# SahakyanLab/GenomeAssembler_dev

Hardware: AMD Instinct MI355X
Metric: k-mers built+scored/sec (higher is better)
Workload: dtype u64 keys / u32 counts / f64 scores; 1 GPU; cfg2 (configs[2]): 100 x 50000 bp segments per GPU, 150 bp reads at 50x, k=31, build + breakage scoring of all contigs; mode=segments, segments_total=100, distinct_kmers_rank0=3843627, parallelism=segments sharded over 1 GPU(s), no collective

## Files before the change

### genomeassembler_dev_amd/csrc/capi.hip

```cpp
#include <algorithm>
#include <atomic>
#include <functional>
#include <memory>
#include <mutex>
#include <new>
#include <thread>

#include "pipeline.h"
#include "scaffolds.h"

struct gasm_strlist {
    std::vector<char> data;
    std::vector<u64> off;
};

struct gasm_contigs {
    std::vector<char> data;
    std::vector<u64> off;
    u64 rows = 0;
    std::vector<u32> perm;
    int words = 1;
    std::vector<u64> dkeys;
    std::vector<u32> dmult;
};
// ... 40 lines not shown
        StepSlot& x = slot[cur];
        if (!x.cx) x.cx = cur ? ctx->lane((size_t)cur) : ctx;
        if (!x.cx) x.cx = ctx;
        return x;
    }
    const StepSlot& S() const { return slot[cur]; }
    bool built = false;
    bool scored = false;
    int score_kmer = 0;
    u32 score_tables = 1;
    int last_k = 0;
    DBuf d_read_start;
    std::vector<u32> h_read_start;
    std::vector<int64_t> h_fx;
    std::vector<u64> h_sim_seg_off;
    DBuf d_rkc;
    bool rkc_checked = false;
    bool rkc_counted = false;
    std::vector<u32> h_rkc;
};

static int batch_queue_score(gasm_batch* b, StepSlot& x) {
    ScoreTable* tbs[GASM_MAX_TABLES];
    b->table_ptrs(tbs);
    return pipeline_score_launch(x.cx, b->rd, x.dp, b->score_kmer, tbs, b->score_tables, false, false, x.ss, &x.bs);
}

static int batch_finish(gasm_batch* b) {
    StepSlot& x = b->S();
    bool rebuilt = false;
    GCHK(pipeline_build_finish(x.cx, b->build_reads(x), x.bs, &rebuilt));
    if (rebuilt) {
        x.paths_ready = false;
        if (b->scored) {
            GCHK(pipeline_contig_paths(x.cx, b->rd, x.bs, x.dp));
            x.paths_ready = true;
            pipeline_contig_paths_host(b->rd, x.bs, x.dp);
            GCHK(batch_queue_score(b, x));
        }
    }
    return GASM_OK;
}

static void strlist_from(const std::vector<std::string>& v, std::vector<char>& data, std::vector<u64>& off) {
    off.assign(v.size() + 1, 0);
    size_t tot = 0;
    for (size_t i = 0; i < v.size(); ++i) { tot += v[i].size(); off[i + 1] = tot; }
    data.resize(tot);
    for (size_t i = 0; i < v.size(); ++i) memcpy(data.data() + off[i], v[i].data(), v[i].size());
}

template <class F>
static int new_batch(gasm_ctx* ctx, u32 n_segments, u64 n_reads, gasm_batch** out, F&& fill) {
    gasm_batch* b = new gasm_batch();
    b->ctx = ctx;
    b->n_segments = n_segments;
    b->n_reads = n_reads;
    const int st = fill(b);
    if (st != GASM_OK) { gasm_batch_free(b); return st; }
    *out = b;
    return GASM_OK;
}

extern "C" {

static int breakscore_impl(gasm_ctx* ctx, DevPaths& dp, const std::function<std::string(u64)>& path_text, uint64_t n_paths, const char* reads,
// ... 972 lines not shown
```

### genomeassembler_dev_amd/csrc/kernels.h

```cpp
#pragma once
#include <hip/hip_runtime.h>
#include <stdint.h>

#include "device_utils.h"
#include "keyops.h"

struct ReadSet {
    const u64* words;
    const u64* read_off;
    const u64* seg_read_off;
    const u32* seg_tile_start;
    const uint4* tile_info;
    u32 fixed_len;
    u32 n_segments;
};

__device__ __forceinline__ void read_span(const ReadSet& rs, u64 r, u64* p0, u32* len) {
    if (rs.fixed_len) { *p0 = rs.read_off ? rs.read_off[r] : r * rs.fixed_len; *len = rs.fixed_len; }
    else { const u64 a = rs.read_off[r]; *p0 = a; *len = (u32)(rs.read_off[r + 1] - a); }
}

struct GraphView {
    const void* dk_key;
    const u32* dstart;
// ... 144 lines not shown
    const u32* elem_skip;
    const u64* elem_pos;
};
__global__ void k_str_bitonic(const u64* words, const u64* off, u32* idx, u32 n_pow2, u32 kk, u32 j, ChainSigs cs);
__global__ void k_str_bitonic_block(const u64* words, const u64* off, u32* idx, u32 n_pow2, u32 kk, u32 j0, ChainSigs cs);
__global__ void k_str_adjacent_eq(const u64* words, const u64* off, const u32* idx, u32 n, u8* same_as_prev, ChainSigs cs);
__global__ void k_unpack_ascii(const u64* words, u64 nbases, u8* out);
__global__ void k_guided_chain(PathSet ps, const unsigned long long* fx, int k, u32* g_next, u32* g_prev, u32* dbg_order);
__global__ void k_asm_match(const u64* cwords, const u64* c_off, u32 n, int k, u8* match, u8* row_any, u8* level_any);
__global__ void k_asm_merge(const u32* perm, u32 rows, u32 n, int k, const u32* clen, const u8* match, const u8* row_any, const u8* level_any,
                            const u64* cwords, const u64* c_off, u32* out_next, u8* out_ov, u32* out_heads, u32* out_nchains, u8* need_host);

__global__ void k_sim_weights(const u64* gwords, const u64* gbase, const u64* woff, u32 n_segments, int kmer, const long long* fixw, u64* w);
template <class T> __global__ void k_seg_scan_incl(T* a, const u64* off);
__global__ void k_sim_draw(const u64* cum, const u64* woff, const u64* doff, const u64* glen, u64 seed, u32 read_len, u32* start, u32* keep);
__global__ void k_sim_compact(const u32* start, const u32* keep, const u32* rank, const u64* doff, const u64* seg_read_off, u32* kept_start);
__global__ void k_sim_extract(const u64* gwords, const u64* gbase, const u64* seg_read_off, const u32* kept_start, u32 read_len, unsigned long long* out);

template <int LS>
__global__ void k_read_kmer_count(const u64* words, const u64* read_off, const u64* seg_read_off, u32 fixed_len, u32 n_segments, u32* out);

struct SeedTable {
    u64* seed;
    u32* gpos;
    const u64* tbl_off;
};
__global__ void k_read_insert(ReadSet rs, SeedTable st, int w);
__global__ void k_path_scan(ReadSet rs, PathSet ps, SeedTable st, const u64* seg_base_off, int w, const u64* first_off, u32* first, u32 seg0,
                            u32 path_lo, u32 path_hi);
__global__ void k_first_to_poscnt(const u32* first, u64 n, u32* poscnt);
#define GASM_SCORE_MAX_TABLES 8
struct FixTables { const long long* p[GASM_SCORE_MAX_TABLES]; };
struct ProbTables { const double* p[GASM_SCORE_MAX_TABLES]; };
template <class K, int T>
__global__ void k_score_reads_graph(ReadSet rs, GraphView gv, const u64* link, const u32* e_cid, PathSet ps, FixTables dfix, int kmer,
                                    u32 reads_per_wg, u32 chunks, u32 lds_paths, u32* cnt, unsigned long long* sum, u64 sum_stride, int verify,
                                    u32* verify_flag);
__global__ void k_levenshtein(PathSet ps, u32 n_paths, const u64* twords, u32 nt, int infix, u8* carry_ws, u64 carry_stride, int32_t* out);
__global__ void k_levenshtein2(PathSet ps, u32 n_paths, const u64* twords, u32 nt, int infix, uint4* carry_ws, u64 carry_stride, int32_t* out);
__global__ void k_score_zero(u32* cnt, unsigned long long* sum, u64 sum_stride, u32 n_tables, const u32* n_paths_p);
__global__ void k_score_finish(PathSet ps, const u32* cnt, const unsigned long long* sum, const long long* dfix, const u64* seg_empty,
                               int kmer, double inv_scale, double* bp_score, double* norm_freq, double* norm_len, int32_t* kmer_breaks,
                               int32_t* seq_len, const u32* n_paths_p);
template <int T>
__global__ void k_path_reduce(PathSet ps, const u32* poscnt, const u32* extra, ProbTables dprob, int kmer, double* bp_score, double* norm_freq,
                              double* norm_len, u64 out_stride, int32_t* kmer_breaks, int32_t* seq_len, u32 n_paths);
__global__ void k_path_freq(PathSet ps, const u32* poscnt, const u32* total, const int32_t* drow, int kmer, u32 n_table,
                            u32* freq_cnt, u32 n_paths);
__global__ void k_ks_genome_hist(const u64* gwords, u64 glen, int kmer, const int32_t* drow, u32* hist);
__global__ void k_path_ks(PathSet ps, const u32* poscnt, const int32_t* drow, int kmer, u32 n_table, const double* pv, const u32* cumy, u32* scratch,
                          double* out, u32 n_paths, const u32* list);
__global__ void k_path_ks2(PathSet ps, const u32* poscnt, const int32_t* drow, int kmer, u32 n_table, const double* pv, const u32* cumy, const u32* run_end,
                           u32* scratch, double* out, u32* flags, u32 n_paths, u32 bins);
__global__ void k_cover_mark(const long long* start, const long long* len, u64 n, long long seq_len, int* diff);
__global__ void k_cover_count(const int* diff, long long seq_len, unsigned long long* covered);
__global__ void k_prob_dist(PathSet ps, const double* dprob, int kmer, const u64* pd_off, double* out, u32 n_paths);

template <class T>
struct XReport {
    T* w;
    u32 W;
    __host__ __device__ T& send_tot(u32 d) const { return w[d]; }
    __host__ __device__ T& recv_tot(u32 d) const { return w[W + d]; }
    __host__ __device__ T& info(u32 j) const { return w[2 * W + j]; }
    __host__ __device__ T& flags() const { return w[2 * W + 4]; }
    __host__ __device__ T& ticket() const { return w[2 * W + 5]; }
    static size_t words(u32 W) { return 2 * (size_t)W + 6; }
};
__global__ void k_x_flag_word(const u32* flags, u32* row_tail);
__global__ void k_x1_plan(const u32* lens_all, u64 stride, u32 nbt, const u32* order, const u32* dst_first, const u32* mine, u32 n_mine, u32 W, u32 r, u32 limit,
                          u64* send_off, u64* send_tot, u64* run_off, u32* run_len, u64* recv_tot, u64* bstart, u32* flags_or);
__global__ void k_x2_fill(u32* G, u32 nbt, const u32* mine, u32 n_mine, const u32* bucket_d, const u32* flags);
__global__ void k_x2_plan(const u32* G, const u16* own1, u32 W, u32 r, u32 gb_lo, u32 n_out, int bbits, const u32* mine, u32 n_mine, const u32* seg_first,
                          u64* send_off, u64* send_tot, u64* run_off, u32* run_len, u64* recv_tot, u64* bstart, u64* info);
__global__ void k_x_report(const u64* send_tot, const u64* recv_tot, u32 W, const u64* info, u32 n_info, const u32* flags_or, u64* report, u64 ticket);
__global__ void k_x_add_u32(u32* acc, const u32* v, u64 n);
// ... 1 lines not shown
```

### genomeassembler_dev_amd/csrc/kernels_score.hip

```cpp
#include "device_utils.h"
#include "kernels.h"

#define GASM_DIRECT_ROWS 87380
__device__ __forceinline__ u32 direct_base(u32 L) { return ((1u << (2 * L)) - 4u) / 3u; }

__device__ __forceinline__ bool break_window(const u64* __restrict__ words, u64 pbase, u32 plen, u32 j, int kmer, u32* idx) {
    const int st = (int)j - kmer / 2;
    const u32 start = st > 0 ? (u32)st : 0u;
    u32 width = 8;
    if (start == 0) {
        if (j == 1) width = 2;
        else if (j == 2) width = 4;
        else if (j == 3) width = 6;
    }
    if (start >= plen) return false;
    const u32 avail = plen - start;
    const u32 wd = width < avail ? width : avail;
    *idx = direct_base(wd) + (u32)kmer_at(words, pbase + start, (int)wd);
    return true;
}

__global__ void __launch_bounds__(GASM_WG) k_read_insert(ReadSet rs, SeedTable st, int w) {
    const u32 seg = blockIdx.y;
    const u64 r = rs.seg_read_off[seg] + (u64)blockIdx.x * GASM_WG + threadIdx.x;
// ... 84 lines not shown
}

template <class K>
__device__ __forceinline__ u64 graph_match(const ReadSet& rs, const GraphView& gv, const u64* __restrict__ link,
                                           const u32* __restrict__ e_cid, const PathSet& ps, u32 seg, u64 r, u32* path, u64* pbeg, u64* pend,
                                           int verify, u32* __restrict__ verify_flag) {
    u64 p0; u32 len;
    read_span(rs, r, &p0, &len);
    if (len < (u32)gv.k) return ~0ull;
    const K key = kmer_key_at<K>(rs.words, p0, gv.k);
    u32 hi;
    const u32 e = graph_lower_bound<K>(gv, seg, key, &hi);
    if (e >= hi || !keq(reinterpret_cast<const K*>(gv.dk_key)[e], key)) return ~0ull;
    const u64 l = link[e];
    const u32 a = (u32)(l >> 32);
    if (a == GASM_NONE32 || !(l & GASM_LINK_DONE)) return ~0ull;
    const u32 c = e_cid[a];
    *path = c;
    const gasm_u64x2 po = load_pair(ps.p_off + c);
    *pbeg = po.x; *pend = po.y;
    const u64 g = po.x + ((u32)l & 0x7FFFFFFFu);
    if (g + len > po.y) return ~0ull;
    if (verify) {
        if (!bases_equal(rs.words, p0, ps.words, g, len)) { if (verify == 1) atomicOr(verify_flag, 1u); return ~0ull; }
    }
    return g;
}

template <class K, int T>
__global__ void __launch_bounds__(GASM_WG) k_score_reads_graph(ReadSet rs, GraphView gv, const u64* __restrict__ link,
                                                               const u32* __restrict__ e_cid, PathSet ps, FixTables dfix, int kmer,
                                                               u32 reads_per_wg, u32 chunks, u32 lds_paths, u32* __restrict__ cnt,
                                                               unsigned long long* __restrict__ sum, u64 sum_stride, int verify,
                                                               u32* __restrict__ verify_flag) {
    extern __shared__ unsigned long long s_sum[];
    u32* s_cnt = reinterpret_cast<u32*>(s_sum + (size_t)T * lds_paths);
    u32 seg, chunk;
    if (!seg_chunk(rs.n_segments, chunks, &seg, &chunk)) return;
    const u64 r0 = rs.seg_read_off[seg] + (u64)chunk * reads_per_wg;
    const u64 rseg_end = rs.seg_read_off[seg + 1];
    if (r0 >= rseg_end) return;
    const u64 r1 = r0 + reads_per_wg < rseg_end ? r0 + reads_per_wg : rseg_end;
    const u32 pfirst = ps.seg_path_off[seg], np = ps.seg_path_off[seg + 1] - pfirst;
    const bool in_lds = np <= lds_paths;
    if (in_lds) for (u32 i = threadIdx.x; i < np; i += GASM_WG) {
#pragma unroll
        for (int t = 0; t < T; ++t) s_sum[(size_t)t * lds_paths + i] = 0;
        s_cnt[i] = 0;
    }
    __syncthreads();
    for (u64 r = r0 + threadIdx.x; r < r1; r += GASM_WG) {
        u32 c = 0;
        u64 pb = 0, pe = 0;
        const u64 g = graph_match<K>(rs, gv, link, e_cid, ps, seg, r, &c, &pb, &pe, verify, verify_flag);
        if (g == ~0ull) continue;
        const u32 plen = (u32)(pe - pb);
        u32 idx = 0;
        const bool hit = break_window(ps.words, pb, plen, (u32)(g - pb), kmer, &idx);
        long long fx[T];
#pragma unroll
        for (int t = 0; t < T; ++t) fx[t] = hit ? dfix.p[t][idx] : 0;
        if (in_lds) {
            atomicAdd(&s_cnt[c - pfirst], 1u);
#pragma unroll
            for (int t = 0; t < T; ++t) atomicAdd(&s_sum[(size_t)t * lds_paths + (c - pfirst)], (unsigned long long)fx[t]);
        } else {
            atomicAdd(&cnt[c], 1u);
#pragma unroll
            for (int t = 0; t < T; ++t) atomicAdd(&sum[(u64)t * sum_stride + c], (unsigned long long)fx[t]);
        }
    }
    __syncthreads();
    if (in_lds) for (u32 i = threadIdx.x; i < np; i += GASM_WG) {
        const u32 c = s_cnt[i];
        if (c) {
            atomicAdd(&cnt[pfirst + i], c);
#pragma unroll
            for (int t = 0; t < T; ++t) atomicAdd(&sum[(u64)t * sum_stride + pfirst + i], s_sum[(size_t)t * lds_paths + i]);
        }
    }
}

#define GASM_INST_SCORE(K, T)                                                                                                         \
    template __global__ void k_score_reads_graph<K, T>(ReadSet, GraphView, const u64*, const u32*, PathSet, FixTables, int, u32, u32, u32, u32*, \
                                                       unsigned long long*, u64, int, u32*);
#define GASM_INST_SCORE_K(K)                                                                                                           \
    GASM_INST_SCORE(K, 1) GASM_INST_SCORE(K, 2) GASM_INST_SCORE(K, 3) GASM_INST_SCORE(K, 4) GASM_INST_SCORE(K, 5) GASM_INST_SCORE(K, 6) \
    GASM_INST_SCORE(K, 7) GASM_INST_SCORE(K, 8)
GASM_INST_SCORE_K(u64)
GASM_INST_SCORE_K(K128)

__global__ void __launch_bounds__(GASM_WG) k_score_zero(u32* __restrict__ cnt, unsigned long long* __restrict__ sum, u64 sum_stride, u32 n_tables,
                                                        const u32* __restrict__ n_paths_p) {
    const u32 n = *n_paths_p;
    for (u32 p = blockIdx.x * GASM_WG + threadIdx.x; p < n; p += gridDim.x * GASM_WG) {
        cnt[p] = 0;
        for (u32 t = 0; t < n_tables; ++t) sum[(u64)t * sum_stride + p] = 0;
    }
}

__global__ void __launch_bounds__(GASM_WG) k_score_finish(PathSet ps, const u32* __restrict__ cnt, const unsigned long long* __restrict__ sum,
                                                          const long long* __restrict__ dfix, const u64* __restrict__ seg_empty,
                                                          int kmer, double inv_scale, double* __restrict__ bp_score,
                                                          double* __restrict__ norm_freq, double* __restrict__ norm_len,
                                                          int32_t* __restrict__ kmer_breaks, int32_t* __restrict__ seq_len,
                                                          const u32* __restrict__ n_paths_p) {
    const u32 n_paths = *n_paths_p;
    for (u32 p = blockIdx.x * GASM_WG + threadIdx.x; p < n_paths; p += gridDim.x * GASM_WG) {
        const u64 pb = ps.p_off[p];
        const u32 len = (u32)(ps.p_off[p + 1] - pb);
        u32 tot = cnt[p];
        long long fs = (long long)sum[p];
        if (seg_empty) {
            const u32 seg = upper_seg<u32>(ps.seg_path_off, ps.n_segments, p);
            const u32 e = (u32)seg_empty[seg];
            if (e) {
                u32 idx;
                tot += e;
                if (break_window(ps.words, pb, len, 0, kmer, &idx)) fs += (long long)e * dfix[idx];
            }
        }
        const double s1 = (double)fs * inv_scale;
        bp_score[p] = s1;
        norm_freq[p] = tot ? s1 / (double)tot : 0.0;
        norm_len[p] = s1 / (double)(int32_t)len;
        kmer_breaks[p] = (int32_t)tot;
        seq_len[p] = (int32_t)len;
    }
}

__device__ __forceinline__ u32 wave_sum_u32(u32 v) {
#pragma unroll
    for (int d = 32; d > 0; d >>= 1) v += __shfl_xor(v, d, 64);
    return v;
}

__device__ __forceinline__ double wave_sum_fixed(double v) {
#pragma unroll
    for (int d = 32; d > 0; d >>= 1) v += __shfl_xor(v, d, 64);
    return v;
}

template <int T>
__global__ void __launch_bounds__(GASM_WG) k_path_reduce(PathSet ps, const u32* __restrict__ poscnt, const u32* __restrict__ extra, ProbTables dprob,
                                                         int kmer, double* __restrict__ bp_score, double* __restrict__ norm_freq,
                                                         double* __restrict__ norm_len, u64 out_stride, int32_t* __restrict__ kmer_breaks,
                                                         int32_t* __restrict__ seq_len, u32 n_paths) {
    __shared__ u32 s_t[4];
    __shared__ double s_a[T][4], s_b[T][4];
    const u32 p = blockIdx.x;
    if (p >= n_paths) return;
    const u32 lane = threadIdx.x & 63, wv = threadIdx.x >> 6;
    const u64 pb = ps.p_off[p];
    const u32 len = (u32)(ps.p_off[p + 1] - pb);
    u32 tsum = 0;
    for (u32 j = threadIdx.x; j < len; j += GASM_WG) tsum += poscnt[pb + j];
    tsum = wave_sum_u32(tsum);
    if (lane == 0) s_t[wv] = tsum;
    __syncthreads();
    const u32 tot = s_t[0] + s_t[1] + s_t[2] + s_t[3] + extra[p];
    const double dtot = (double)tot;
    double s1[T], s2[T];
// ... 622 lines not shown
```

### genomeassembler_dev_amd/csrc/pipeline.h

```cpp
#pragma once
#include "gasm_internal.h"
#include "kernels.h"

template <class K> struct KeyTag { using type = K; };
template <class F> static inline int with_key(int words, F&& f) { return words == 1 ? f(KeyTag<u64>{}) : f(KeyTag<K128>{}); }
#define GLAUNCH_K(ctx, words, name, kern, grid, block, shmem, ...)          \
    GCHK(with_key(words, [&](auto _tag) -> int {                            \
        using K = typename decltype(_tag)::type;                            \
        GLAUNCH(ctx, name, kern, grid, block, shmem, __VA_ARGS__);          \
        return GASM_OK;                                                     \
    }))

struct DevReads {
    u32 n_segments = 0;
    u64 n_reads = 0, total_bases = 0;
    u32 fixed_len = 0;
    u32 min_len = 0, max_len = 0;
    u64 n_empty = 0;
    std::vector<u64> h_read_off;
    std::vector<u64> h_seg_read_off;
    std::vector<u64> h_seg_empty;
    bool positioned = false;
    int sim_shift = 52;
    u64 upload_id = 0;
// ... 87 lines not shown
    std::vector<u32> h_dk_cnt, h_nxt;
    std::vector<u64> h_solid_before, h_solid_after, h_spectrum;
    bool spectrum_queued = false;
    std::vector<u8> h_eflag;
    std::vector<char> h_contigs;
    bool fetched_distinct = false, fetched_contigs = false;
    void release();
};

struct ScoreTable {
    DBuf d_prob, d_row, d_fix;
    std::vector<double> h_prob;
    std::vector<double> h_row_prob;
    double h_absmax = 0;
    bool h_finite = false;
    int fix_shift = -1;
    u32 n_table = 0;
    int fixed_shift(u64 max_terms) const;
    int set_fixed(gasm_ctx* ctx, int shift);
    int set(gasm_ctx* ctx, const char* bp_kmer, const u64* bp_off, u64 n_table, const double* bp_prob);
    int set_standard(gasm_ctx* ctx, const double* table69904);
    void release();
};

struct ScoreState {
    DBuf d_tbl_off, d_seed, d_gpos, d_poscnt, d_total, d_out_f64, d_out_i32, d_freq, d_pd_off, d_pd, d_seg_empty, d_fxsum, d_first, d_first_off;
    std::vector<u64> h_toff;
    u32 n_paths = 0, n_table = 0;
    u32 n_tables = 1;
    size_t stride = 1;
    const BuildState* graph = nullptr;
    bool want_freq = false, want_pd = false, launched = false;
    bool verify = false;
    std::vector<double> h_bp, h_nf, h_nl, h_freq, h_pd;
    std::vector<int32_t> h_breaks, h_len;
    std::vector<u64> h_pd_off;
    bool valid = false;
    void release();
};

int pipeline_build(gasm_ctx* ctx, DevReads& rd, int k, u64 genome_len_hint, BuildState& bs, u32 min_count = 1, u32 strands = 1, u32 tip_len = 0,
                   u32 tip_rounds = 0);
int pipeline_build_finish(gasm_ctx* ctx, DevReads& rd, BuildState& bs, bool* rebuilt);
int pipeline_build_finish_n(gasm_ctx* ctx, DevReads* rd, u32 n_segments, BuildState& bs, bool* rebuilt);
enum : u32 { GASM_RUNG_EXACT = 1, GASM_RUNG_TABLE = 2, GASM_RUNG_BBITS = 4, GASM_RUNG_MULTI = 8, GASM_RUNG_ALL = 15 };
bool build_next_config(u32 ovf, u32 rungs, int words, int bb_cap, bool& single_pass, bool& small_tbl, int& bbits, bool& multi_pass);
void pipeline_build_plan(const DevReads& rd, const BuildState& bs, int32_t* row);
int plan_build(gasm_ctx* ctx, DevReads& rd, int k, u64 hint, BuildState& bs);
void distinct_caps(BuildState& bs, u32 n_segments);
int launch_distinct(gasm_ctx* ctx, DevReads& rd, BuildState& bs);
int launch_graph(gasm_ctx* ctx, u32 n_segments, BuildState& bs);
int pipeline_fetch_distinct(gasm_ctx* ctx, DevReads& rd, BuildState& bs);
int pipeline_fetch_contigs(gasm_ctx* ctx, DevReads& rd, BuildState& bs);
int pipeline_fetch_solid_stats(gasm_ctx* ctx, DevReads& rd, BuildState& bs);
int pipeline_fetch_tip_stats(gasm_ctx* ctx, DevReads& rd, BuildState& bs);
int pipeline_kmer_spectrum(gasm_ctx* ctx, DevReads& rd, BuildState& bs);
int pipeline_fetch_kmer_spectrum(gasm_ctx* ctx, DevReads& rd, BuildState& bs);
int pipeline_fetch_contig_twins(gasm_ctx* ctx, DevReads& rd, BuildState& bs);
int pipeline_fetch_graph(gasm_ctx* ctx, DevReads& rd, BuildState& bs);
int pipeline_contig_paths(gasm_ctx* ctx, const DevReads& rd, const BuildState& bs, DevPaths& dp);
void pipeline_contig_paths_host(const DevReads& rd, const BuildState& bs, DevPaths& dp);
int pipeline_score_launch(gasm_ctx* ctx, DevReads& rd, DevPaths& dp, int kmer, ScoreTable* const* tbs, u32 n_tables, bool want_freq,
                          bool want_pd, ScoreState& ss, const BuildState* graph);
int pipeline_score_fetch(gasm_ctx* ctx, ScoreState& ss);
bool pipeline_score_uses_graph(const DevReads& rd, const BuildState& graph, ScoreTable* const* tbs, u32 n_tables);
int pipeline_ks(gasm_ctx* ctx, DevPaths& dp, ScoreState& ss, const ScoreTable& tb, const char* genome, u64 genome_len, int kmer, std::vector<double>& ks);
// ... 16 lines not shown
```

### genomeassembler_dev_amd/csrc/pipeline.hip

```cpp
#include <atomic>
#include <chrono>
#include <thread>
#include "pipeline.h"

#include <algorithm>
#include <cmath>

__global__ void k_set_u64(u64* p, u64 v) { *p = v; }

__global__ void k_add_empty_reads(PathSet ps, const u64* __restrict__ seg_empty, u32* __restrict__ poscnt, u32* __restrict__ total) {
    const u32 seg = blockIdx.y;
    const u32 p = ps.seg_path_off[seg] + blockIdx.x * GASM_WG + threadIdx.x;
    if (p >= ps.seg_path_off[seg + 1]) return;
    const u32 e = (u32)seg_empty[seg];
    if (!e) return;
    if (ps.p_off[p + 1] > ps.p_off[p]) poscnt[ps.p_off[p]] += e;
    else total[p] += e;
}

struct Knobs {
    int dedup_tbl = 0, dbg_dedup = 0, padm = -1, scatter_wgs = 8, hist_wgs = 64, rank_rounds = 18, bbits_add = 0, ruler_shift = 0;
    bool rank_global = false, sync_build = false;
    int dedup_warm = 0;
    const char* stamps = nullptr;
// ... 366 lines not shown
    }
    total_bases = h_p_off[np];
    if (total_bases >= 0xFFFFFFF0ull) { gasm_set_error("paths exceed 2^32 bases"); return GASM_ERR_CAPACITY; }
    h_seg_path_off = {0u, np};
    DBuf ascii;
    GCHK(h2d(ctx, ascii, data + off[0], total_bases));
    int st = pack_from_device_ascii(ctx, ascii.as<u8>());
    ascii.release();
    GCHK(st);
    return upload_dirs(ctx);
}

PathSet DevPaths::view() const {
    PathSet v;
    v.words = d_words.as<u64>();
    v.p_off = b_p_off ? b_p_off : d_p_off.as<u64>();
    v.seg_path_off = b_seg_path_off ? b_seg_path_off : d_seg_path_off.as<u32>();
    v.n_segments = n_segments;
    return v;
}

void DevPaths::release() { d_words.release(); d_p_off.release(); d_seg_path_off.release(); d_seg_base_off.release(); }

void BuildState::release() {
    for (DBuf* b : {&d_solid_removed, &d_tip_stats, &d_spectrum, &d_twin, &d_keys, &d_keys2, &d_mult, &d_hist, &d_toff, &d_tcnt, &d_fdir, &d_bstart, &d_bucket_d, &d_dstart, &d_flags, &d_dk_key, &d_dk_cnt,
                    &d_eflag, &d_nxt, &d_link, &d_clen, &d_ecid, &d_ecoff, &d_rtab, &d_seg_cbases, &d_seg_cstart,
                    &d_seg_bstart, &d_c_off, &d_contig_ascii})
        b->release();
    part_valid = false;
    if (h_report) { (void)hipHostFree(h_report); h_report = nullptr; h_report_words = 0; }
}

void ScoreState::release() {
    for (DBuf* b : {&d_tbl_off, &d_seed, &d_gpos, &d_poscnt, &d_total, &d_out_f64, &d_out_i32, &d_freq, &d_pd_off, &d_pd, &d_seg_empty, &d_fxsum, &d_first, &d_first_off}) b->release();
}

static int ensure_lds_attrs(gasm_ctx* ctx) {
    if (ctx->lds_attrs_set) return GASM_OK;
#define GASM_LDS_ATTR(kern, bytes) HIPCHK(hipFuncSetAttribute(reinterpret_cast<const void*>(kern), hipFuncAttributeMaxDynamicSharedMemorySize, bytes));
#define GASM_SCORE_LDS_ATTR(T) GASM_LDS_ATTR((k_score_reads_graph<K, T>), GASM_SCORE_PATH_CAP * 12)
    for (int words = 1; words <= 2; ++words)
        GCHK(with_key(words, [&](auto tag) -> int {
            using K = typename decltype(tag)::type;
            GASM_LDS_ATTR(k_bucket_scatter<K>, 160 * 1024) GASM_LDS_ATTR(k_bucket_partition<K>, 160 * 1024) GASM_LDS_ATTR(k_tile_hist<K>, 160 * 1024)
            GASM_SCORE_LDS_ATTR(1) GASM_SCORE_LDS_ATTR(2) GASM_SCORE_LDS_ATTR(3) GASM_SCORE_LDS_ATTR(4) GASM_SCORE_LDS_ATTR(5) GASM_SCORE_LDS_ATTR(6) GASM_SCORE_LDS_ATTR(7) GASM_SCORE_LDS_ATTR(8)
            return GASM_OK;
        }));
    GASM_LDS_ATTR(k_rank_lds, 160 * 1024 - 64)
#undef GASM_SCORE_LDS_ATTR
#undef GASM_LDS_ATTR
    ctx->lds_attrs_set = true;
    return GASM_OK;
}

void distinct_caps(BuildState& bs, u32 S) {
    const u64 limit = bs.multi_pass ? GASM_BUCKET_MAX : bs.small_tbl ? GASM_TBL_LIMIT / 2 : GASM_TBL_LIMIT;
    const u64 per_seg = ((u64)1 << bs.bbits) * limit;
    const u64 all = bs.k < 16 ? ((u64)1 << (2 * bs.k)) : ~(u64)0;
    bs.D_cap = 0; bs.maxD_cap = 0;
    for (u32 s = 0; s < S; ++s) {
        const u64 c = std::min(std::min(bs.h_seg_nk[s], per_seg), all);
        bs.D_cap += c;
        bs.maxD_cap = std::max(bs.maxD_cap, c);
    }
}

static int launch_graph_dense(gasm_ctx* ctx, u32 S, BuildState& bs, bool last_pass);
// ... 794 lines not shown
    HIPCHK(hipMemcpyAsync(&c, cov.p, 8, hipMemcpyDeviceToHost, ctx->stream));
    HIPCHK(hipStreamSynchronize(ctx->stream));
    *percent = (1.0 - (double)(seq_len - (long long)c) / (double)seq_len) * 100.0;
    return GASM_OK;
}

static u64 max_seg_reads(const DevReads& rd) {
    u64 m = 0;
    for (u32 s = 0; s < rd.n_segments; ++s) m = std::max(m, rd.h_seg_read_off[s + 1] - rd.h_seg_read_off[s]);
    return m;
}

static_assert(GASM_SCORE_MAX_TABLES == GASM_MAX_TABLES, "kernels.h and gasm.h disagree on the number of tables");

#define GASM_TABLES_SWITCH(T, CASE)                                                                                      \
    switch (T) {                                                                                                         \
        case 1: CASE(1); break; case 2: CASE(2); break; case 3: CASE(3); break; case 4: CASE(4); break; case 5: CASE(5); break;  \
        case 6: CASE(6); break; case 7: CASE(7); break; default: CASE(8); break;                                         \
    }

static int score_launch_graph(gasm_ctx* ctx, DevReads& rd, DevPaths& dp, int kmer, ScoreTable* const* tbs, u32 T, ScoreState& ss,
                              const BuildState& graph) {
    GasmRange range("gasm:score (graph-indexed)");
    GCHK(ensure_lds_attrs(ctx));
    const u32 S = rd.n_segments;
    const size_t PC = (size_t)graph.D_cap + 1;
    ss.stride = PC;
    ss.graph = &graph;
    ss.n_paths = 0;
    const size_t fx_off = (PC * 4 + 15) & ~(size_t)15;
    GCHK(ss.d_total.ensure(fx_off + PC * 8 * T));
    GCHK(ss.d_out_f64.ensure(PC * 8 * 3 * T));
    GCHK(ss.d_out_i32.ensure(PC * 4 * 2));
    unsigned long long* const d_fx = reinterpret_cast<unsigned long long*>(static_cast<char*>(ss.d_total.p) + fx_off);
    const u32* const n_paths_p = graph.d_seg_cstart.as<u32>() + S;
    const u64 p_est = graph.have_actual ? std::max<u64>(graph.n_contigs, 1) : (u64)S * 256;
    const u32 grid_p = (u32)std::max<u64>(1, std::min<u64>(ceil_div_u64(p_est, GASM_WG), (u64)ctx->n_cu * 8));
    GLAUNCH(ctx, "k_score_zero", k_score_zero, dim3(grid_p), dim3(GASM_WG), 0, ss.d_total.as<u32>(), d_fx, (u64)PC, T, n_paths_p);
    const PathSet ps = dp.view();
    const GraphView gv = graph_view(graph);
    const u64 max_reads = max_seg_reads(rd);
    FixTables ft = {};
    for (u32 t = 0; t < T; ++t) {
        GCHK(tbs[t]->set_fixed(ctx, tbs[t]->fixed_shift(max_reads)));
        ft.p[t] = tbs[t]->d_fix.as<long long>();
    }
    const int verify = (graph.min_count > 1 || graph.tip_len) ? 2 : env_int("GASM_SCORE_VERIFY", 0) != 0 ? 1 : 0;
    ss.verify = verify == 1;
    const u32 reads_per_wg = 256;
    const u32 rchunks = (u32)ceil_div_u64(max_reads, reads_per_wg);
    u32 lds_paths = std::min<u32>(std::max<u32>(graph.have_actual ? graph.paths_est : 1024u, 1u), (u32)(GASM_SCORE_PATH_CAP * 12 / (4 + 8 * T)));
    if (const int cap = env_int("GASM_DBG_SCORE_LDS_PATHS", 0)) lds_paths = std::min<u32>(lds_paths, (u32)std::max(1, cap));
    const size_t lds_bytes = (size_t)lds_paths * (4 + 8 * (size_t)T);
#define GASM_LAUNCH_SCORE(TT)                                                                                                                       \
    GLAUNCH_K(ctx, graph.words, "k_score_reads_graph", (k_score_reads_graph<K, TT>), seg_grid(rchunks, S), dim3(GASM_WG), lds_bytes, rd.view(), gv, \
              graph.d_link.as<u64>(), graph.d_ecid.as<u32>(), ps, ft, kmer, reads_per_wg, rchunks, lds_paths, ss.d_total.as<u32>(), d_fx, (u64)PC,  \
              verify, graph.d_flags.as<u32>() + GASM_FLAG_SCORE_MISMATCH)
    GASM_TABLES_SWITCH(T, GASM_LAUNCH_SCORE)
#undef GASM_LAUNCH_SCORE
    int32_t* o_br = ss.d_out_i32.as<int32_t>();
    int32_t* o_ln = o_br + PC;
    const u64* d_se = nullptr;
    if (rd.n_empty) { GCHK(h2d(ctx, ss.d_seg_empty, rd.h_seg_empty.data(), (size_t)S * 8)); d_se = ss.d_seg_empty.as<u64>(); }
    for (u32 t = 0; t < T; ++t) {
        double* o_bp = ss.d_out_f64.as<double>() + (size_t)t * 3 * PC;
        GLAUNCH(ctx, "k_score_finish", k_score_finish, dim3(grid_p), dim3(GASM_WG), 0, ps, ss.d_total.as<u32>(), d_fx + (size_t)t * PC, ft.p[t], d_se, kmer,
                std::ldexp(1.0, -tbs[t]->fix_shift), o_bp, o_bp + PC, o_bp + 2 * PC, o_br, o_ln, n_paths_p);
    }
    ss.h_pd_off.clear();
    ss.launched = true;
    return GASM_OK;
}

bool pipeline_score_uses_graph(const DevReads& rd, const BuildState& graph, ScoreTable* const* tbs, u32 T) {
    if (!(graph.n_kmers > 0 && rd.n_reads > rd.n_empty && rd.min_len >= (u32)graph.k)) return false;
    const u64 max_reads = max_seg_reads(rd);
    for (u32 t = 0; t < T; ++t) if (tbs[t]->fixed_shift(max_reads) < 0) return false;
    return true;
}

static int score_positions(gasm_ctx* ctx, DevReads& rd, DevPaths& dp, ScoreState& ss, u32 n_tables) {
    ss.n_paths = dp.n_paths;
    const u32 S = rd.n_segments, P = dp.n_paths;
    const u64 TB = dp.total_bases;
    ss.stride = (size_t)P + 1;
    GCHK(ss.d_poscnt.ensure((TB + 1) * 4));
    GCHK(ss.d_total.ensure(((size_t)P + 1) * 4));
    GCHK(ss.d_out_f64.ensure(((size_t)P + 1) * 8 * 3 * n_tables));
    GCHK(ss.d_out_i32.ensure(((size_t)P + 1) * 4 * 2));
    HIPCHK(hipMemsetAsync(ss.d_poscnt.p, 0, (TB + 1) * 4, ctx->stream));
    HIPCHK(hipMemsetAsync(ss.d_total.p, 0, ((size_t)P + 1) * 4, ctx->stream));
    const PathSet ps = dp.view();
    const int w = (int)std::min<u32>(32, rd.min_len);
    if (P && TB && rd.n_reads > rd.n_empty && w >= 1) {
        std::vector<u64>& toff = ss.h_toff;
        toff.assign((size_t)S + 1, 0);
        std::vector<u64> foff((size_t)S + 1, 0);
        u64 max_bases = 0, max_reads = 0;
        for (u32 s = 0; s < S; ++s) {
            const u64 nbases = dp.h_seg_base_off[s + 1] - dp.h_seg_base_off[s];
            const u64 nreads = rd.h_seg_read_off[s + 1] - rd.h_seg_read_off[s];
// ... 177 lines not shown
```

### genomeassembler_dev_amd/csrc/pool.hip

```cpp
#include <algorithm>

#include "pool.h"

static int read_lens(gasm_pool* p, u32 n) {
    p->h_len.assign(n, 0);
    if (n) HIPCHK(hipMemcpyAsync(p->h_len.data(), p->bs.d_bucket_d.p, (size_t)n * 4, hipMemcpyDeviceToHost, p->ctx->stream));
    u32 ovf = 0;
    HIPCHK(hipMemcpyAsync(&ovf, p->bs.d_flags.as<u32>() + GASM_FLAG_OVERFLOW, 4, hipMemcpyDeviceToHost, p->ctx->stream));
    HIPCHK(hipStreamSynchronize(p->ctx->stream));
    return (int)(ovf & (GASM_OVF_TABLE | GASM_OVF_REGION));
}

int pool_empty_runs(gasm_pool* p) {
    gasm_ctx* ctx = p->ctx;
    BuildState& bs = p->bs;
    GCHK(bs.d_bucket_d.ensure(((size_t)p->n_runs + 2) * 4));
    GCHK(bs.d_bstart.ensure(((size_t)p->n_runs + 1) * 8));
    GCHK(bs.d_keys.ensure(64)); GCHK(bs.d_mult.ensure(64));
    HIPCHK(hipMemsetAsync(bs.d_bucket_d.p, 0, ((size_t)p->n_runs + 2) * 4, ctx->stream));
    bs.part_valid = false;
    HIPCHK(hipMemsetAsync(bs.d_bstart.p, 0, ((size_t)p->n_runs + 1) * 8, ctx->stream));
    HIPCHK(hipMemsetAsync(bs.d_flags.p, 0, GASM_FLAG_BYTES, ctx->stream));
    return GASM_OK;
}
// ... 49 lines not shown
    if (S == 0) return GASM_OK;
    GCHK(bs.d_dstart.ensure(((size_t)p->n_runs + 2) * 4));
    GLAUNCH(ctx, "k_scan_excl", k_scan_excl<u32>, dim3(1), dim3(1024), 0, bs.d_bucket_d.as<u32>(), bs.d_dstart.as<u32>(), p->n_runs);
    GCHK(launch_graph(ctx, S, bs));
    return GASM_OK;
}

int pool_score_launch(gasm_pool* p, int kmer, const double* table, bool wait_for_build) {
    if (!p->graphed || !p->reads_set) { gasm_set_error("scoring needs the rank's graph and the reads of its segments first"); return GASM_ERR_STATE; }
    gasm_ctx* ctx = p->ctx;
    if (!p->table_set || memcmp(p->table_copy.data(), table, GASM_TABLE_ROWS * sizeof(double)) != 0) {
        GCHK(p->tb.set_standard(ctx, table));
        p->table_copy.assign(table, table + GASM_TABLE_ROWS);
        p->table_set = true;
    }
    ScoreTable* const tb = &p->tb;
    const bool through_graph = p->n_local && pipeline_score_uses_graph(p->own, p->bs, &tb, 1);
    if (wait_for_build || !through_graph) GCHK(pipeline_build_finish_n(ctx, nullptr, p->n_local, p->bs, nullptr));
    if (!p->paths_ready) {
        GCHK(pipeline_contig_paths(ctx, p->own, p->bs, p->dp));
        p->paths_ready = true;
    }
    if (!p->bs.pending) pipeline_contig_paths_host(p->own, p->bs, p->dp);
    GCHK(pipeline_score_launch(ctx, p->own, p->dp, kmer, &tb, 1, false, false, p->ss, &p->bs));
    p->scored = true; p->score_kmer = kmer;
    return GASM_OK;
}

int pool_finish(gasm_pool* p) {
    bool rebuilt = false;
    GCHK(pipeline_build_finish_n(p->ctx, nullptr, p->n_local, p->bs, &rebuilt));
    if (rebuilt && p->scored) {
        p->paths_ready = false;
        GCHK(pool_score_launch(p, p->score_kmer, p->table_copy.data(), true));
    }
    return GASM_OK;
}

extern "C" {

int gasm_pool_create(gasm_ctx* ctx, const char* reads, uint64_t n_reads, uint32_t fixed_len, const uint64_t* seg_read_off,
                     uint32_t n_segments, gasm_pool** out) {
    API_GUARD_BEGIN
    if (!ctx || !out) { gasm_set_error("gasm_pool_create: null argument"); return GASM_ERR_INVALID; }
    *out = nullptr;
    if (fixed_len == 0) { gasm_set_error("pooled builds take fixed-length reads"); return GASM_ERR_INVALID; }
    gasm_pool* p = new gasm_pool();
    p->ctx = ctx;
    const int st = p->rd.upload(ctx, reads, nullptr, n_reads, fixed_len, seg_read_off, n_segments);
    if (st != GASM_OK) { gasm_pool_free(p); return st; }
    *out = p;
    return GASM_OK;
    API_GUARD_END
}

void gasm_pool_free(gasm_pool* p) {
    if (!p) return;
    if (p->ctx) { (void)hipSetDevice(p->ctx->device); (void)hipStreamSynchronize(p->ctx->stream); }
    p->rd.release(); p->bs.release(); p->own.release(); p->dp.release(); p->tb.release(); p->ss.release();
    p->d_list.release(); p->d_off.release(); p->d_roff.release(); p->d_rlen.release();
    delete p;
}

int gasm_pool_key_words(const gasm_pool* p) { return p ? p->bs.words : 0; }

int gasm_pool_local_runs(gasm_pool* p, int k, int bbits, const uint32_t** run_len) {
// ... 247 lines not shown
```

Baseline: 223.6 billion k-mers/s.

## Fuse score zeroing and finish into graph scoring kernel via last-block ticket

Removes the separate k_score_zero and per-table k_score_finish launches. The last workgroup of each segment, chosen by an atomic ticket counter, now computes the per-path outputs and resets the accumulators to zero inside k_score_reads_graph. The accumulators live in a dedicated buffer that is memset only when it is reallocated or marked dirty after a rebuild, which saves launches and a full pass over the path arrays. In exchange the code relies on cross-workgroup memory ordering through relaxed atomics plus an explicit vmcnt wait, and the per-segment finish work is serialized onto one workgroup.

```diff
diff --git a/genomeassembler_dev_amd/csrc/capi.hip b/genomeassembler_dev_amd/csrc/capi.hip
--- a/genomeassembler_dev_amd/csrc/capi.hip
+++ b/genomeassembler_dev_amd/csrc/capi.hip
@@ -96,6 +96,7 @@
     GCHK(pipeline_build_finish(x.cx, b->build_reads(x), x.bs, &rebuilt));
     if (rebuilt) {
         x.paths_ready = false;
+        x.ss.acc_dirty = true;
         if (b->scored) {
             GCHK(pipeline_contig_paths(x.cx, b->rd, x.bs, x.dp));
             x.paths_ready = true;
diff --git a/genomeassembler_dev_amd/csrc/kernels.h b/genomeassembler_dev_amd/csrc/kernels.h
--- a/genomeassembler_dev_amd/csrc/kernels.h
+++ b/genomeassembler_dev_amd/csrc/kernels.h
@@ -200,16 +200,21 @@
 #define GASM_SCORE_MAX_TABLES 8
 struct FixTables { const long long* p[GASM_SCORE_MAX_TABLES]; };
 struct ProbTables { const double* p[GASM_SCORE_MAX_TABLES]; };
+struct ScoreFinish {
+    double inv_scale[GASM_SCORE_MAX_TABLES];
+    double* out_f64;
+    int32_t* kmer_breaks;
+    int32_t* seq_len;
+    unsigned long long* fx_out;
+    const u64* seg_empty;
+    u32* ticket;
+};
 template <class K, int T>
 __global__ void k_score_reads_graph(ReadSet rs, GraphView gv, const u64* link, const u32* e_cid, PathSet ps, FixTables dfix, int kmer,
                                     u32 reads_per_wg, u32 chunks, u32 lds_paths, u32* cnt, unsigned long long* sum, u64 sum_stride, int verify,
-                                    u32* verify_flag);
+                                    u32* verify_flag, ScoreFinish fin);
 __global__ void k_levenshtein(PathSet ps, u32 n_paths, const u64* twords, u32 nt, int infix, u8* carry_ws, u64 carry_stride, int32_t* out);
 __global__ void k_levenshtein2(PathSet ps, u32 n_paths, const u64* twords, u32 nt, int infix, uint4* carry_ws, u64 carry_stride, int32_t* out);
-__global__ void k_score_zero(u32* cnt, unsigned long long* sum, u64 sum_stride, u32 n_tables, const u32* n_paths_p);
-__global__ void k_score_finish(PathSet ps, const u32* cnt, const unsigned long long* sum, const long long* dfix, const u64* seg_empty,
-                               int kmer, double inv_scale, double* bp_score, double* norm_freq, double* norm_len, int32_t* kmer_breaks,
-                               int32_t* seq_len, const u32* n_paths_p);
 template <int T>
 __global__ void k_path_reduce(PathSet ps, const u32* poscnt, const u32* extra, ProbTables dprob, int kmer, double* bp_score, double* norm_freq,
                               double* norm_len, u64 out_stride, int32_t* kmer_breaks, int32_t* seq_len, u32 n_paths);
diff --git a/genomeassembler_dev_amd/csrc/kernels_score.hip b/genomeassembler_dev_amd/csrc/kernels_score.hip
--- a/genomeassembler_dev_amd/csrc/kernels_score.hip
+++ b/genomeassembler_dev_amd/csrc/kernels_score.hip
@@ -140,102 +140,101 @@
                                                                const u32* __restrict__ e_cid, PathSet ps, FixTables dfix, int kmer,
                                                                u32 reads_per_wg, u32 chunks, u32 lds_paths, u32* __restrict__ cnt,
                                                                unsigned long long* __restrict__ sum, u64 sum_stride, int verify,
-                                                               u32* __restrict__ verify_flag) {
+                                                               u32* __restrict__ verify_flag, ScoreFinish fin) {
     extern __shared__ unsigned long long s_sum[];
+    __shared__ u32 s_last;
     u32* s_cnt = reinterpret_cast<u32*>(s_sum + (size_t)T * lds_paths);
     u32 seg, chunk;
     if (!seg_chunk(rs.n_segments, chunks, &seg, &chunk)) return;
     const u64 r0 = rs.seg_read_off[seg] + (u64)chunk * reads_per_wg;
     const u64 rseg_end = rs.seg_read_off[seg + 1];
-    if (r0 >= rseg_end) return;
-    const u64 r1 = r0 + reads_per_wg < rseg_end ? r0 + reads_per_wg : rseg_end;
     const u32 pfirst = ps.seg_path_off[seg], np = ps.seg_path_off[seg + 1] - pfirst;
-    const bool in_lds = np <= lds_paths;
-    if (in_lds) for (u32 i = threadIdx.x; i < np; i += GASM_WG) {
-#pragma unroll
-        for (int t = 0; t < T; ++t) s_sum[(size_t)t * lds_paths + i] = 0;
-        s_cnt[i] = 0;
-    }
+    if (r0 < rseg_end) {
+        const u64 r1 = r0 + reads_per_wg < rseg_end ? r0 + reads_per_wg : rseg_end;
+        const bool in_lds = np <= lds_paths;
+        if (in_lds) for (u32 i = threadIdx.x; i < np; i += GASM_WG) {
+#pragma unroll
+            for (int t = 0; t < T; ++t) s_sum[(size_t)t * lds_paths + i] = 0;
+            s_cnt[i] = 0;
+        }
+        __syncthreads();
+        for (u64 r = r0 + threadIdx.x; r < r1; r += GASM_WG) {
+            u32 c = 0;
+            u64 pb = 0, pe = 0;
+            const u64 g = graph_match<K>(rs, gv, link, e_cid, ps, seg, r, &c, &pb, &pe, verify, verify_flag);
+            if (g == ~0ull) continue;
+            const u32 plen = (u32)(pe - pb);
+            u32 idx = 0;
+            const bool hit = break_window(ps.words, pb, plen, (u32)(g - pb), kmer, &idx);
+            long long fx[T];
+#pragma unroll
+            for (int t = 0; t < T; ++t) fx[t] = hit ? dfix.p[t][idx] : 0;
+            if (in_lds) {
+                atomicAdd(&s_cnt[c - pfirst], 1u);
+#pragma unroll
+                for (int t = 0; t < T; ++t) atomicAdd(&s_sum[(size_t)t * lds_paths + (c - pfirst)], (unsigned long long)fx[t]);
+            } else {
+                atomicAdd(&cnt[c], 1u);
+#pragma unroll
+                for (int t = 0; t < T; ++t) atomicAdd(&sum[(u64)t * sum_stride + c], (unsigned long long)fx[t]);
+            }
+        }
+        __syncthreads();
+        if (in_lds) for (u32 i = threadIdx.x; i < np; i += GASM_WG) {
+            const u32 c = s_cnt[i];
+            if (c) {
+                atomicAdd(&cnt[pfirst + i], c);
+#pragma unroll
+                for (int t = 0; t < T; ++t) atomicAdd(&sum[(u64)t * sum_stride + pfirst + i], s_sum[(size_t)t * lds_paths + i]);
+            }
+        }
+    }
+    __asm__ volatile("s_waitcnt vmcnt(0)" ::: "memory");
     __syncthreads();
-    for (u64 r = r0 + threadIdx.x; r < r1; r += GASM_WG) {
-        u32 c = 0;
-        u64 pb = 0, pe = 0;
-        const u64 g = graph_match<K>(rs, gv, link, e_cid, ps, seg, r, &c, &pb, &pe, verify, verify_flag);
-        if (g == ~0ull) continue;
-        const u32 plen = (u32)(pe - pb);
-        u32 idx = 0;
-        const bool hit = break_window(ps.words, pb, plen, (u32)(g - pb), kmer, &idx);
-        long long fx[T];
-#pragma unroll
-        for (int t = 0; t < T; ++t) fx[t] = hit ? dfix.p[t][idx] : 0;
-        if (in_lds) {
-            atomicAdd(&s_cnt[c - pfirst], 1u);
-#pragma unroll
-            for (int t = 0; t < T; ++t) atomicAdd(&s_sum[(size_t)t * lds_paths + (c - pfirst)], (unsigned long long)fx[t]);
-        } else {
-            atomicAdd(&cnt[c], 1u);
-#pragma unroll
-            for (int t = 0; t < T; ++t) atomicAdd(&sum[(u64)t * sum_stride + c], (unsigned long long)fx[t]);
-        }
-    }
+    if (threadIdx.x == 0) s_last = __hip_atomic_fetch_add(&fin.ticket[seg], 1u, __ATOMIC_RELAXED, __HIP_MEMORY_SCOPE_AGENT) == chunks - 1 ? 1u : 0u;
     __syncthreads();
-    if (in_lds) for (u32 i = threadIdx.x; i < np; i += GASM_WG) {
-        const u32 c = s_cnt[i];
-        if (c) {
-            atomicAdd(&cnt[pfirst + i], c);
-#pragma unroll
-            for (int t = 0; t < T; ++t) atomicAdd(&sum[(u64)t * sum_stride + pfirst + i], s_sum[(size_t)t * lds_paths + i]);
-        }
+    if (!s_last) return;
+    if (threadIdx.x == 0) __hip_atomic_store(&fin.ticket[seg], 0u, __ATOMIC_RELAXED, __HIP_MEMORY_SCOPE_AGENT);
+    const u32 n_empty = fin.seg_empty ? (u32)fin.seg_empty[seg] : 0u;
+    for (u32 p = pfirst + threadIdx.x; p < pfirst + np; p += GASM_WG) {
+        const u64 pb = ps.p_off[p];
+        const u32 len = (u32)(ps.p_off[p + 1] - pb);
+        const u32 hits = __hip_atomic_load(&cnt[p], __ATOMIC_RELAXED, __HIP_MEMORY_SCOPE_AGENT);
+        unsigned long long raw[T];
+#pragma unroll
+        for (int t = 0; t < T; ++t) raw[t] = hits ? __hip_atomic_load(&sum[(u64)t * sum_stride + p], __ATOMIC_RELAXED, __HIP_MEMORY_SCOPE_AGENT) : 0ull;
+        if (hits) {
+            __hip_atomic_store(&cnt[p], 0u, __ATOMIC_RELAXED, __HIP_MEMORY_SCOPE_AGENT);
+#pragma unroll
+            for (int t = 0; t < T; ++t) __hip_atomic_store(&sum[(u64)t * sum_stride + p], 0ull, __ATOMIC_RELAXED, __HIP_MEMORY_SCOPE_AGENT);
+        }
+        u32 tot = hits, idx = 0;
+        bool e_hit = false;
+        if (n_empty) { tot += n_empty; e_hit = break_window(ps.words, pb, len, 0, kmer, &idx); }
+#pragma unroll
+        for (int t = 0; t < T; ++t) {
+            fin.fx_out[(u64)t * sum_stride + p] = raw[t];
+            long long fs = (long long)raw[t];
+            if (e_hit) fs += (long long)n_empty * dfix.p[t][idx];
+            const double s1 = (double)fs * fin.inv_scale[t];
+            double* const o_bp = fin.out_f64 + (u64)t * 3 * sum_stride;
+            o_bp[p] = s1;
+            o_bp[sum_stride + p] = tot ? s1 / (double)tot : 0.0;
+            o_bp[2 * sum_stride + p] = s1 / (double)(int32_t)len;
+        }
+        fin.kmer_breaks[p] = (int32_t)tot;
+        fin.seq_len[p] = (int32_t)len;
     }
 }
 
 #define GASM_INST_SCORE(K, T)                                                                                                         \
     template __global__ void k_score_reads_graph<K, T>(ReadSet, GraphView, const u64*, const u32*, PathSet, FixTables, int, u32, u32, u32, u32*, \
-                                                       unsigned long long*, u64, int, u32*);
+                                                       unsigned long long*, u64, int, u32*, ScoreFinish);
 #define GASM_INST_SCORE_K(K)                                                                                                           \
     GASM_INST_SCORE(K, 1) GASM_INST_SCORE(K, 2) GASM_INST_SCORE(K, 3) GASM_INST_SCORE(K, 4) GASM_INST_SCORE(K, 5) GASM_INST_SCORE(K, 6) \
     GASM_INST_SCORE(K, 7) GASM_INST_SCORE(K, 8)
 GASM_INST_SCORE_K(u64)
 GASM_INST_SCORE_K(K128)
-
-__global__ void __launch_bounds__(GASM_WG) k_score_zero(u32* __restrict__ cnt, unsigned long long* __restrict__ sum, u64 sum_stride, u32 n_tables,
-                                                        const u32* __restrict__ n_paths_p) {
-    const u32 n = *n_paths_p;
-    for (u32 p = blockIdx.x * GASM_WG + threadIdx.x; p < n; p += gridDim.x * GASM_WG) {
-        cnt[p] = 0;
-        for (u32 t = 0; t < n_tables; ++t) sum[(u64)t * sum_stride + p] = 0;
-    }
-}
-
-__global__ void __launch_bounds__(GASM_WG) k_score_finish(PathSet ps, const u32* __restrict__ cnt, const unsigned long long* __restrict__ sum,
-                                                          const long long* __restrict__ dfix, const u64* __restrict__ seg_empty,
-                                                          int kmer, double inv_scale, double* __restrict__ bp_score,
-                                                          double* __restrict__ norm_freq, double* __restrict__ norm_len,
-                                                          int32_t* __restrict__ kmer_breaks, int32_t* __restrict__ seq_len,
-                                                          const u32* __restrict__ n_paths_p) {
-    const u32 n_paths = *n_paths_p;
-    for (u32 p = blockIdx.x * GASM_WG + threadIdx.x; p < n_paths; p += gridDim.x * GASM_WG) {
-        const u64 pb = ps.p_off[p];
-        const u32 len = (u32)(ps.p_off[p + 1] - pb);
-        u32 tot = cnt[p];
-        long long fs = (long long)sum[p];
-        if (seg_empty) {
-            const u32 seg = upper_seg<u32>(ps.seg_path_off, ps.n_segments, p);
-            const u32 e = (u32)seg_empty[seg];
-            if (e) {
-                u32 idx;
-                tot += e;
-                if (break_window(ps.words, pb, len, 0, kmer, &idx)) fs += (long long)e * dfix[idx];
-            }
-        }
-        const double s1 = (double)fs * inv_scale;
-        bp_score[p] = s1;
-        norm_freq[p] = tot ? s1 / (double)tot : 0.0;
-        norm_len[p] = s1 / (double)(int32_t)len;
-        kmer_breaks[p] = (int32_t)tot;
-        seq_len[p] = (int32_t)len;
-    }
-}
 
 __device__ __forceinline__ u32 wave_sum_u32(u32 v) {
 #pragma unroll
diff --git a/genomeassembler_dev_amd/csrc/pipeline.h b/genomeassembler_dev_amd/csrc/pipeline.h
--- a/genomeassembler_dev_amd/csrc/pipeline.h
+++ b/genomeassembler_dev_amd/csrc/pipeline.h
@@ -143,6 +143,10 @@
     const BuildState* graph = nullptr;
     bool want_freq = false, want_pd = false, launched = false;
     bool verify = false;
+    DBuf d_acc;
+    const void* acc_zero_p = nullptr;
+    size_t acc_zero_cap = 0;
+    bool acc_dirty = false;
     std::vector<double> h_bp, h_nf, h_nl, h_freq, h_pd;
     std::vector<int32_t> h_breaks, h_len;
     std::vector<u64> h_pd_off;
diff --git a/genomeassembler_dev_amd/csrc/pipeline.hip b/genomeassembler_dev_amd/csrc/pipeline.hip
--- a/genomeassembler_dev_amd/csrc/pipeline.hip
+++ b/genomeassembler_dev_amd/csrc/pipeline.hip
@@ -422,7 +422,8 @@
 }
 
 void ScoreState::release() {
-    for (DBuf* b : {&d_tbl_off, &d_seed, &d_gpos, &d_poscnt, &d_total, &d_out_f64, &d_out_i32, &d_freq, &d_pd_off, &d_pd, &d_seg_empty, &d_fxsum, &d_first, &d_first_off}) b->release();
+    for (DBuf* b : {&d_tbl_off, &d_seed, &d_gpos, &d_poscnt, &d_total, &d_out_f64, &d_out_i32, &d_freq, &d_pd_off, &d_pd, &d_seg_empty, &d_fxsum, &d_first, &d_first_off, &d_acc}) b->release();
+    acc_zero_p = nullptr; acc_zero_cap = 0;
 }
 
 static int ensure_lds_attrs(gasm_ctx* ctx) {
@@ -1283,19 +1284,32 @@
     GCHK(ss.d_total.ensure(fx_off + PC * 8 * T));
     GCHK(ss.d_out_f64.ensure(PC * 8 * 3 * T));
     GCHK(ss.d_out_i32.ensure(PC * 4 * 2));
-    unsigned long long* const d_fx = reinterpret_cast<unsigned long long*>(static_cast<char*>(ss.d_total.p) + fx_off);
-    const u32* const n_paths_p = graph.d_seg_cstart.as<u32>() + S;
-    const u64 p_est = graph.have_actual ? std::max<u64>(graph.n_contigs, 1) : (u64)S * 256;
-    const u32 grid_p = (u32)std::max<u64>(1, std::min<u64>(ceil_div_u64(p_est, GASM_WG), (u64)ctx->n_cu * 8));
-    GLAUNCH(ctx, "k_score_zero", k_score_zero, dim3(grid_p), dim3(GASM_WG), 0, ss.d_total.as<u32>(), d_fx, (u64)PC, T, n_paths_p);
+    const size_t cnt_off = ((size_t)S * 4 + 15) & ~(size_t)15, sum_off = cnt_off + fx_off;
+    GCHK(ss.d_acc.ensure(sum_off + PC * 8 * T));
+    if (ss.acc_dirty || ss.acc_zero_p != ss.d_acc.p || ss.acc_zero_cap != ss.d_acc.cap) {
+        ss.acc_zero_p = nullptr;
+        HIPCHK(hipMemsetAsync(ss.d_acc.p, 0, ss.d_acc.cap, ctx->stream));
+        ss.acc_zero_p = ss.d_acc.p; ss.acc_zero_cap = ss.d_acc.cap;
+    }
+    ss.acc_dirty = true;
+    u32* const d_cnt = reinterpret_cast<u32*>(static_cast<char*>(ss.d_acc.p) + cnt_off);
+    unsigned long long* const d_sum = reinterpret_cast<unsigned long long*>(static_cast<char*>(ss.d_acc.p) + sum_off);
     const PathSet ps = dp.view();
     const GraphView gv = graph_view(graph);
     const u64 max_reads = max_seg_reads(rd);
     FixTables ft = {};
+    ScoreFinish fin = {};
     for (u32 t = 0; t < T; ++t) {
         GCHK(tbs[t]->set_fixed(ctx, tbs[t]->fixed_shift(max_reads)));
         ft.p[t] = tbs[t]->d_fix.as<long long>();
-    }
+        fin.inv_scale[t] = std::ldexp(1.0, -tbs[t]->fix_shift);
+    }
+    fin.out_f64 = ss.d_out_f64.as<double>();
+    fin.kmer_breaks = ss.d_out_i32.as<int32_t>();
+    fin.seq_len = fin.kmer_breaks + PC;
+    fin.fx_out = reinterpret_cast<unsigned long long*>(static_cast<char*>(ss.d_total.p) + fx_off);
+    fin.ticket = ss.d_acc.as<u32>();
+    if (rd.n_empty) { GCHK(h2d(ctx, ss.d_seg_empty, rd.h_seg_empty.data(), (size_t)S * 8)); fin.seg_empty = ss.d_seg_empty.as<u64>(); }
     const int verify = (graph.min_count > 1 || graph.tip_len) ? 2 : env_int("GASM_SCORE_VERIFY", 0) != 0 ? 1 : 0;
     ss.verify = verify == 1;
     const u32 reads_per_wg = 256;
@@ -1305,19 +1319,11 @@
     const size_t lds_bytes = (size_t)lds_paths * (4 + 8 * (size_t)T);
 #define GASM_LAUNCH_SCORE(TT)                                                                                                                       \
     GLAUNCH_K(ctx, graph.words, "k_score_reads_graph", (k_score_reads_graph<K, TT>), seg_grid(rchunks, S), dim3(GASM_WG), lds_bytes, rd.view(), gv, \
-              graph.d_link.as<u64>(), graph.d_ecid.as<u32>(), ps, ft, kmer, reads_per_wg, rchunks, lds_paths, ss.d_total.as<u32>(), d_fx, (u64)PC,  \
-              verify, graph.d_flags.as<u32>() + GASM_FLAG_SCORE_MISMATCH)
+              graph.d_link.as<u64>(), graph.d_ecid.as<u32>(), ps, ft, kmer, reads_per_wg, rchunks, lds_paths, d_cnt, d_sum, (u64)PC, verify,        \
+              graph.d_flags.as<u32>() + GASM_FLAG_SCORE_MISMATCH, fin)
     GASM_TABLES_SWITCH(T, GASM_LAUNCH_SCORE)
 #undef GASM_LAUNCH_SCORE
-    int32_t* o_br = ss.d_out_i32.as<int32_t>();
-    int32_t* o_ln = o_br + PC;
-    const u64* d_se = nullptr;
-    if (rd.n_empty) { GCHK(h2d(ctx, ss.d_seg_empty, rd.h_seg_empty.data(), (size_t)S * 8)); d_se = ss.d_seg_empty.as<u64>(); }
-    for (u32 t = 0; t < T; ++t) {
-        double* o_bp = ss.d_out_f64.as<double>() + (size_t)t * 3 * PC;
-        GLAUNCH(ctx, "k_score_finish", k_score_finish, dim3(grid_p), dim3(GASM_WG), 0, ps, ss.d_total.as<u32>(), d_fx + (size_t)t * PC, ft.p[t], d_se, kmer,
-                std::ldexp(1.0, -tbs[t]->fix_shift), o_bp, o_bp + PC, o_bp + 2 * PC, o_br, o_ln, n_paths_p);
-    }
+    ss.acc_dirty = false;
     ss.h_pd_off.clear();
     ss.launched = true;
     return GASM_OK;
diff --git a/genomeassembler_dev_amd/csrc/pool.hip b/genomeassembler_dev_amd/csrc/pool.hip
--- a/genomeassembler_dev_amd/csrc/pool.hip
+++ b/genomeassembler_dev_amd/csrc/pool.hip
@@ -105,6 +105,7 @@
     GCHK(pipeline_build_finish_n(p->ctx, nullptr, p->n_local, p->bs, &rebuilt));
     if (rebuilt && p->scored) {
         p->paths_ready = false;
+        p->ss.acc_dirty = true;
         GCHK(pool_score_launch(p, p->score_kmer, p->table_copy.data(), true));
     }
     return GASM_OK;
```

Measured after the change: 223.3 billion k-mers/s. About the same (-0.1%).
